# bharathikannann/Depth-Fusion-in-Transformer-Based-Video-Object-Detection

Hardware: AMD Instinct MI355X
Metric: frames/sec at 800x1333 RGB-D, TransVOD++ Late-Fusion (higher is better)
Workload: dtype f32; 1 GPU; TransVOD++ LateFusion, 32-frame 800x1333 RGB-D clip, all-current mode (R=31), L=1 DC5 (S=4200), 300 queries, 3 classes; frames_per_gpu=32, frames_per_gpu_per_clip=32, micro_batch=32, two_stream_overlap=False, clip_pipeline=True, pipeline_lanes=2, hip_hw_queues=4, hip_graphs=False

## Files before the change

### depth-fusion-in-transformer-based-video-object-detection_amd/csrc/conv_tile.hip

```cpp
#include "dfx_common.h"
#include "dfx_conv.h"
#include <type_traits>

namespace {

using f32x16 = __attribute__((ext_vector_type(16))) float;
using f32x4 = __attribute__((ext_vector_type(4))) float;
using i32x4 = __attribute__((ext_vector_type(4))) int;

constexpr int kTH = 8, kTW = 32, kThreads = 512, kMaxStage = 9;

struct TileArgs {
    const float *X, *Wp, *bias;
    float *Y;
    int Ci, H, W, Co, Ho, Wo, Kpad, K, KH, KW, stride, pad, act;
    long strideX, strideY;
    int TX, TY;
    long tiles;
    int IH, IW, PW;
    int nstage;
    unsigned xbytes;
};

__device__ __forceinline__ float activate(float v, int act)
// ... 13 lines not shown
    int *const koff = reinterpret_cast<int *>(smem + 32 * MT * LDA);
    float *const img = smem + 32 * MT * LDA + g.Kpad;
    float *const bl = img + 2 * IMG;

    const int tid = threadIdx.x, lane = tid & 63, wave = tid >> 6;
    const int half = lane >> 5, c = lane & 31;
    const int s = g.stride, PW = g.PW, PWH = PW >> 1;
    const int HW = g.H * g.W;

    for (int f = tid; f < 32 * MT * (g.Kpad / 4); f += kThreads) {
        const int row = f / (g.Kpad / 4), kq = f - row * (g.Kpad / 4);
        f32x4 v = {0.f, 0.f, 0.f, 0.f};
        if (row < g.Co) v = *reinterpret_cast<const f32x4 *>(g.Wp + (long)row * g.Kpad + kq * 4);
        *reinterpret_cast<f32x4 *>(As + row * LDA + kq * 4) = v;
    }
    for (int i = tid; i < 32 * MT; i += kThreads) bl[i] = (g.bias && i < g.Co) ? g.bias[i] : 0.f;
    for (int k = tid; k < g.Kpad; k += kThreads) {
        int o = 0;
        if (k < g.K) {
            const int tap = k / g.Ci, ci = k - tap * g.Ci, ky = tap / g.KW, kx = tap - ky * g.KW;
            o = ci * g.IH * PW + ky * PW + (s == 2 ? (kx & 1) * PWH + (kx >> 1) : kx);
        }
        koff[k] = o;
    }
    const int py = wave, px = c;
    const int pixbase = py * s * PW + px;

    int s_lds[NS], s_rx[NS];
    const int nel = g.Ci * g.IH * g.IW;
#pragma unroll
    for (int u = 0; u < NS; ++u) {
        const int e = tid + u * kThreads;
        const int ci = e / (g.IH * g.IW), rem = e - ci * (g.IH * g.IW), r = rem / g.IW, x = rem - r * g.IW;
        s_lds[u] = e < nel ? ci * g.IH * PW + r * PW + (s == 2 ? (x & 1) * PWH + (x >> 1) : x) : -1;
        s_rx[u] = (ci << 16) | (r << 8) | x;
    }
    const __amdgpu_buffer_rsrc_t rsX = __builtin_amdgcn_make_buffer_rsrc(const_cast<float *>(g.X), 0, (int)g.xbytes, 0x00020000);
    constexpr unsigned kOut = 0xFFFFFFFCu;
    float st[NS];
    const int G = (int)gridDim.x;
    const int d_n = G / (g.TY * g.TX), d_ty = (G - d_n * (g.TY * g.TX)) / g.TX, d_tx = G - d_n * (g.TY * g.TX) - d_ty * g.TX;
    struct Pos { int n, ty, tx; };
    auto advance = [&](Pos p) {
        p.tx += d_tx;
        if (p.tx >= g.TX) { p.tx -= g.TX; p.ty += 1; }
        p.ty += d_ty;
        if (p.ty >= g.TY) { p.ty -= g.TY; p.n += 1; }
        p.n += d_n;
        return p;
    };
    auto stage_load = [&](const Pos &p) {
        const int iy0 = p.ty * kTH * s - g.pad, ix0 = p.tx * kTW * s - g.pad;
        const int base = (int)((long)p.n * g.strideX) + iy0 * g.W + ix0;
        const bool inside = iy0 >= 0 && ix0 >= 0 && iy0 + g.IH <= g.H && ix0 + g.IW <= g.W;
        auto loads = [&](auto checked_tag) {
            constexpr bool CHECKED = decltype(checked_tag)::value;
#pragma unroll
            for (int u = 0; u < NS; ++u) {
                int pk = s_rx[u];
                asm volatile("" : "+v"(pk));
                const int x = pk & 255, r = (pk >> 8) & 255, ci = pk >> 16;
                unsigned off = (unsigned)(base + (ci * HW + r * g.W + x)) * 4u;
                bool bad = s_lds[u] < 0;
                if (CHECKED) bad = bad | ((unsigned)(ix0 + x) >= (unsigned)g.W) | ((unsigned)(iy0 + r) >= (unsigned)g.H);
                off = bad ? kOut : off;
                st[u] = __builtin_bit_cast(float, __builtin_amdgcn_raw_buffer_load_b32(rsX, off, 0, 0));
            }
        };
        if (inside) loads(std::false_type{}); else loads(std::true_type{});
    };
    auto stage_store = [&](int buf) {
        float *dst = img + buf * IMG;
#pragma unroll
        for (int u = 0; u < NS; ++u)
            if (s_lds[u] >= 0) dst[s_lds[u]] = st[u];
    };

    Pos cur;
    {
        const int t0 = (int)blockIdx.x, per = g.TY * g.TX;
        cur.n = t0 / per;
        cur.ty = (t0 - cur.n * per) / g.TX;
        cur.tx = t0 - cur.n * per - cur.ty * g.TX;
    }
    long t = blockIdx.x;
    if (t < g.tiles) {
        stage_load(cur);
        stage_store(0);
    }
    __syncthreads();
    const int nsteps = g.Kpad / 16;
    const unsigned P4 = (unsigned)(g.Ho * g.Wo) * 4u;
    int buf = 0;
    for (; t < g.tiles; t += G) {
        const bool more = t + G < g.tiles;
        const Pos nxt = advance(cur);
        if (more) stage_load(nxt);
        f32x16 acc[MT];
#pragma unroll
        for (int i = 0; i < MT; ++i)
#pragma unroll
            for (int r = 0; r < 16; ++r) acc[i][r] = bl[i * 32 + (r & 3) + 8 * (r >> 2) + 4 * half];
        const float *im = img + buf * IMG + pixbase;
#pragma unroll 1
        for (int ks = 0; ks < nsteps; ++ks) {
            const i32x4 o0 = *reinterpret_cast<const i32x4 *>(koff + ks * 16 + half * 4);
            const i32x4 o1 = *reinterpret_cast<const i32x4 *>(koff + ks * 16 + 8 + half * 4);
            f32x4 af[2][MT];
#pragma unroll
            for (int j = 0; j < 2; ++j)
#pragma unroll
                for (int i = 0; i < MT; ++i)
                    af[j][i] = *reinterpret_cast<const f32x4 *>(As + (i * 32 + c) * LDA + ks * 16 + j * 8 + half * 4);
            float bv[8];
#pragma unroll
            for (int q = 0; q < 4; ++q) {
                bv[q] = im[o0[q]];
                bv[4 + q] = im[o1[q]];
            }
#pragma unroll
            for (int q = 0; q < 8; ++q)
#pragma unroll
                for (int i = 0; i < MT; ++i)
                    acc[i] = __builtin_amdgcn_mfma_f32_32x32x2f32(af[q >> 2][i][q & 3], bv[q], acc[i], 0, 0, 0);
        }
        {
            const int oy = cur.ty * kTH + py, ox = cur.tx * kTW + px;
            const __amdgpu_buffer_rsrc_t rsY = __builtin_amdgcn_make_buffer_rsrc(g.Y + (long)cur.n * g.strideY, 0, (int)((unsigned)g.Co * P4), 0x00020000);
            const unsigned pix = (oy < g.Ho && ox < g.Wo) ? (unsigned)(oy * g.Wo + ox) * 4u + (unsigned)(4 * half) * P4 : 0x80000000u;
            auto write = [&](auto act_tag) {
                constexpr int ACT = decltype(act_tag)::value;
#pragma unroll
                for (int i = 0; i < MT; ++i)
#pragma unroll
                    for (int r = 0; r < 16; ++r) {
                        const int cr = i * 32 + (r & 3) + 8 * (r >> 2);
                        float v = acc[i][r];
                        if (ACT == DFX_ACT_RELU) asm("v_max_f32 %0, 0, %1" : "=v"(v) : "v"(v));
                        if (ACT == DFX_ACT_GELU) v = activate(v, DFX_ACT_GELU);
                        __builtin_amdgcn_raw_buffer_store_b32(__builtin_bit_cast(unsigned, v), rsY, pix, (unsigned)cr * P4, 0);
                    }
            };
            if (g.act == DFX_ACT_RELU) write(std::integral_constant<int, DFX_ACT_RELU>{});
            else if (g.act == DFX_ACT_GELU) write(std::integral_constant<int, DFX_ACT_GELU>{});
            else write(std::integral_constant<int, DFX_ACT_NONE>{});
        }
        if (more) stage_store(buf ^ 1);
        __syncthreads();
        buf ^= 1;
        cur = nxt;
    }
}

}

extern "C" int dfx_conv2d_tile_fits(int Ci, int Co, int KH, int KW, int stride, int dilation)
{
    if (Ci <= 0 || Co <= 0 || KH <= 0 || KW <= 0) return 0;
    const int K = Ci * KH * KW, Kpad = (K + 15) / 16 * 16;
    const int IH = (kTH - 1) * stride + KH, IW = (kTW - 1) * stride + KW;
    return (stride == 1 || stride == 2) && dilation == 1 && Co <= 64 && Kpad <= 160 && IH <= 255 && IW <= 255 &&
           (Ci * IH * IW + kThreads - 1) / kThreads <= kMaxStage;
}

extern "C" int dfx_conv2d_tile_f32(const float *x, const float *wp, const float *bias, float *y, int N, int Ci, int H, int W,
                                   int Co, int Ho, int Wo, int Kpad, int KH, int KW, int stride, int pad, int act,
                                   long x_image_stride, void *stream)
{
    if (N < 0 || Ci <= 0 || H <= 0 || W <= 0 || Co <= 0 || Ho < 0 || Wo < 0 || Kpad <= 0 || stride <= 0 || pad < 0 || KH <= 0 ||
        KW <= 0)
        return dfx::fail(DFX_EINVAL, "conv2d_tile: bad dimension");
    if ((long)N * Ho * Wo == 0) return DFX_OK;
    if (!x || !wp || !y) return dfx::fail(DFX_EINVAL, "conv2d_tile: null pointer");
    if (act < 0 || act > 2) return dfx::fail(DFX_EINVAL, "conv2d_tile: unknown activation");
    const int K = Ci * KH * KW;
    if (!dfx_conv2d_tile_fits(Ci, Co, KH, KW, stride, 1) || Kpad != (K + 15) / 16 * 16 || !dfx::aligned16(wp))
        return dfx::fail(DFX_EINVAL, "conv2d_tile: covers stride 1 / 2, Co <= 64, Ci * KH * KW <= 160 (padded to 16), wp 16-byte aligned");
    if ((Ho - 1) * stride - pad + KH > H + pad || (Wo - 1) * stride - pad + KW > W + pad)
        return dfx::fail(DFX_EINVAL, "conv2d_tile: output size does not match the input geometry");
    TileArgs g{};
    g.X = x; g.Wp = wp; g.bias = bias; g.Y = y;
    g.Ci = Ci; g.H = H; g.W = W; g.Co = Co; g.Ho = Ho; g.Wo = Wo; g.Kpad = Kpad; g.K = K; g.KH = KH; g.KW = KW;
    g.stride = stride; g.pad = pad; g.act = act;
    g.strideX = x_image_stride > 0 ? x_image_stride : (long)Ci * H * W;
    g.strideY = (long)Co * Ho * Wo;
    const long xel = (long)(N - 1) * g.strideX + (long)Ci * H * W;
    if (xel * 4 >= (1L << 32) - 8 || (long)Co * Ho * Wo * 4 >= (1L << 32))
        return dfx::fail(DFX_ERANGE, "conv2d_tile: the input batch or one output image exceeds 4 GiB (split the batch)");
    g.xbytes = (unsigned)(xel * 4);
    g.TY = (Ho + kTH - 1) / kTH;
    g.TX = (Wo + kTW - 1) / kTW;
    g.tiles = (long)N * g.TY * g.TX;
    g.IH = (kTH - 1) * stride + KH;
    g.IW = (kTW - 1) * stride + KW;
    g.PW = stride == 2 ? 2 * ((g.IW + 1) / 2) : g.IW;
    g.nstage = (Ci * g.IH * g.IW + kThreads - 1) / kThreads;
    const int MT = Co <= 32 ? 1 : 2;
    const size_t lds = (size_t)(32 * MT * (Kpad + 4) + Kpad + 2 * Ci * g.IH * g.PW + 32 * MT) * 4;
    if (lds > 160 * 1024) return dfx::fail(DFX_EINVAL, "conv2d_tile: the staged tile does not fit the LDS");
    hipStream_t st = static_cast<hipStream_t>(stream);
    static std::mutex mu;
    static bool raised_on[64] = {false};
    int dev = 0;
    (void)hipGetDevice(&dev);
    {
        std::lock_guard<std::mutex> lock(mu);
        if (!raised_on[dev & 63]) {
            if (hipFuncSetAttribute(reinterpret_cast<const void *>(&conv_tile_kernel<1, 3>), hipFuncAttributeMaxDynamicSharedMemorySize, 160 * 1024) != hipSuccess ||
                hipFuncSetAttribute(reinterpret_cast<const void *>(&conv_tile_kernel<1, kMaxStage>), hipFuncAttributeMaxDynamicSharedMemorySize, 160 * 1024) != hipSuccess ||
                hipFuncSetAttribute(reinterpret_cast<const void *>(&conv_tile_kernel<2, kMaxStage>), hipFuncAttributeMaxDynamicSharedMemorySize, 160 * 1024) != hipSuccess)
                return dfx::fail(DFX_ELAUNCH, "conv2d_tile: cannot raise the dynamic LDS limit");
            raised_on[dev & 63] = true;
        }
    }
    static int ncu = 0;
    if (ncu == 0) {
        int n = 0;
        if (hipDeviceGetAttribute(&n, hipDeviceAttributeMultiprocessorCount, dev) != hipSuccess || n < 8) n = 256;
        ncu = n;
    }
    const long per_cu = lds * 4 <= 160 * 1024 ? 4 : lds * 2 <= 160 * 1024 ? 2 : 1;
    const long grid = g.tiles < ncu * per_cu ? g.tiles : ncu * per_cu;
    const long flops = 2L * Co * Kpad * Ho * Wo * N;
    if (MT == 1 && g.nstage <= 3) dfx::launch_timed(flops, -4, 16, conv_tile_kernel<1, 3>, dim3((unsigned)grid), dim3(kThreads), lds, st, g);
    else if (MT == 1) dfx::launch_timed(flops, -4, 16, conv_tile_kernel<1, kMaxStage>, dim3((unsigned)grid), dim3(kThreads), lds, st, g);
    else dfx::launch_timed(flops, -4, 16, conv_tile_kernel<2, kMaxStage>, dim3((unsigned)grid), dim3(kThreads), lds, st, g);
    return dfx::check_launch("conv_tile_kernel");
}
```

### depth-fusion-in-transformer-based-video-object-detection_amd/dfx/_lib.py

```python
import ctypes
import os

_HERE = os.path.dirname(os.path.abspath(__file__))
_SO = os.environ.get("DFX_LIBRARY") or os.path.join(_HERE, "libdfx.so")
_lib = None

_i, _l, _p = ctypes.c_int, ctypes.c_long, ctypes.c_void_p
_DIMS = [_i] * 7

SIGNATURES = {
    "dfx_msda_forward_f32": [_p] * 5 + _DIMS + [_p, _p],
    "dfx_msda_forward_f64": [_p] * 5 + _DIMS + [_p, _p],
    "dfx_msda_backward_f32": [_p] * 6 + _DIMS + [_p, _p, _p, _p],
    "dfx_msda_backward_f64": [_p] * 6 + _DIMS + [_p, _p, _p, _p],
    "dfx_msda_forward_bf16": [_p] * 5 + _DIMS + [_p, _p],
    "dfx_msda_forward_f16": [_p] * 5 + _DIMS + [_p, _p],
    "dfx_msda_backward_bf16": [_p] * 6 + _DIMS + [_p, _p, _p, _p],
    "dfx_msda_backward_f16": [_p] * 6 + _DIMS + [_p, _p, _p, _p],
    "dfx_msda_fused_forward_f32": [_p, _p, _p, _p, _i, _i, _p, _l, _p, _l] + _DIMS + [_p, _p],
    "dfx_msda_fused_backward_f32": [_p, _p, _p, _p, _i, _p, _l, _p, _l, _p] + _DIMS + [_p, _p, _l, _p, _l, _p, _p],
    "dfx_msda_level_grad_value_f32": [_p, _i, _p, _l, _p, _l, _p, _i, _i, _i, _i, _p, _p],
    "dfx_profile_enable": [_i],
    "dfx_tuning_reload": [],
    "dfx_profile_drain": [_p, _p, _p, _p, _i],
    "dfx_msda_fused_level_fits": [_i, _i],
    "dfx_msda_fused_level_forward_f32": [_p, _p, _i, _p, _p, _p, _i, _i, _i, _i, _p, _p],
    "dfx_mha_f32": [_p, _l, _l, _p, _l, _l, _p, _l, _l, _p, _l, _l, _i, _i, _i, _i, ctypes.c_float, _p],
    "dfx_mha_train_forward_f32": [_p, _l, _l] * 4 + [_p, _p, _i, _i, _i, _i, ctypes.c_float, _p],
    "dfx_mha_backward_f32": [_p, _l, _l] * 5 + [_p, _p] + [_p, _l, _l] * 3 + [_i, _i, _i, _i, ctypes.c_float, _p],
    "dfx_roi_align_nchw_f32": [_p, _p] + [_i] * 7 + [ctypes.c_float, _i, _i, _p, _p],
    "dfx_roi_align_nhwc_f32": [_p, _p] + [_i] * 7 + [ctypes.c_float, _i, _i, _p, _p],
    "dfx_roi_align_backward_nchw_f32": [_p, _p] + [_i] * 7 + [ctypes.c_float, _i, _i, _p, _p],
    "dfx_roi_align_backward_nhwc_f32": [_p, _p] + [_i] * 7 + [ctypes.c_float, _i, _i, _p, _p],
    "dfx_dynamic_conv_f32": [_p, _p, _l, _p, _p, _p, _p, _p, _i, _i, _i, _i, ctypes.c_float, _p],
    "dfx_dynamic_conv_backward_f32": [_p, _p, _p, _l, _p, _p, _p, _p, _p, _p, _l, _p, _p, _i, _i, _i, _i, ctypes.c_float, _p],
    "dfx_preprocess_u8_f32": [_p, _i, _i, _i, _p, _p, _i, _p, _p, _i, _i, _i, _p, _p, _p, _l, _i, _i, _p, _p],
    "dfx_gemm_f32": [_p, _p, _l, _l, _p, _l, _l, _i, _p, _i, _p, _l, _l, _p, _l, _p, _l, _l, _i, _i, _i, _i, _i, _i, _l, _l, _p],
    "dfx_gemm_splitk_f32": [_p, _l, _p, _l, _i, _p, _i, _p, _l, _p, _l, _i, _i, _i, _i, _i, _p, _p],
    "dfx_conv1x1_pair_f32": [_p, _p, _l, _i, _p, _l, _i, _p, _p, _l, _i, _i, _i, _i, _p],
    "dfx_conv1x1_chain_f32": [_p, _p, _l, _i, _p, _l, _i, _p, _p, _l, _p, _l, _p, _p, _p, _l, _i, _i, _i, _i, _i, _p],
    "dfx_bias_act_nchw_f32": [_p, _p, _p, _p, _i, _i, _l, _i, _p],
    "dfx_bias_relu_maxpool_f32": [_p, _p, _p, _i, _i, _i, _i, _p],
    "dfx_add_layernorm_f32": [_p, _p, _p, _p, _p, _l, _i, ctypes.c_float, _p],
    "dfx_box_refine_f32": [_p, _p, _i, _p, _l, ctypes.c_float, _p],
    "dfx_group_norm_f32": [_p, _p, _p, _p, _p, _i, _i, _l, _i, ctypes.c_float, _i, _p],
    "dfx_conv2d_igemm_f32": [_p, _p, _p, _p, _p] + [_i] * 14 + [_l, _p],
    "dfx_conv2d_tile_fits": [_i] * 6,
    "dfx_conv2d_tile_f32": [_p, _p, _p, _p] + [_i] * 13 + [_l, _p],
    "dfx_conv3x3_wino_f32": [_p, _p, _p, _p] + [_i] * 7 + [_p],
    "dfx_wino_weights_f32": [_p, _p, _p, _i, _i, _p],
}


class LevelLayout(ctypes.Structure):
    _fields_ = [(n, ctypes.c_long) for n in (
        "value_frame", "value_token", "value_head", "value_oct", "value_chunk",
        "off_row", "off_head", "logit_row", "logit_head",
        "out_row", "out_head", "out_oct", "out_chunk")]


def library_path():
    return _SO


def load():
    global _lib
    if _lib is None:
        if not os.path.exists(_SO):
            raise RuntimeError(
                f"{_SO} is missing: the HIP extension has not been built "
                "(run `python __graft_entry__.py build` or `make -C <pkg>/csrc`). "
                "There is no CPU or PyTorch fallback for this operator.")
        lib = ctypes.CDLL(_SO)
        for name, argtypes in SIGNATURES.items():
            fn = getattr(lib, name)
            fn.argtypes = argtypes
            fn.restype = ctypes.c_int
        lib.dfx_abi_version.restype = ctypes.c_int
        lib.dfx_last_error.restype = ctypes.c_char_p
        _lib = lib
    return _lib


def abi_version():
    return load().dfx_abi_version()


def check(rc, what):
    if rc != 0:
        msg = load().dfx_last_error().decode() or f"error code {rc}"
        raise RuntimeError(f"{what}: {msg}")
```

### depth-fusion-in-transformer-based-video-object-detection_amd/dfx/ops.py

```python
import ctypes
import os

import torch

from . import _lib

_SUFFIX = {torch.float32: "f32", torch.float64: "f64"}
_HALF_SUFFIX = {torch.bfloat16: "bf16", torch.float16: "f16"}
ACT = {None: 0, "none": 0, "relu": 1, "gelu": 2}

USE_LEVEL_KERNEL = os.environ.get("DFX_MSDA_LEVEL", "1") == "1"
LEVEL_MIN_QUERIES = 1024
USE_LEVEL_BWD = os.environ.get("DFX_MSDA_LEVEL_BWD", "1") != "0"
LEVEL_BWD_MIN_QUERIES = 9600
USE_TILE_CONV = os.environ.get("DFX_TILE_CONV", "1") == "1"

def profile_start():
    _lib.load().dfx_profile_enable(1)


def reload_tuning():
    _lib.load().dfx_tuning_reload()


# ... 713 lines not shown
    @staticmethod
    def forward(ctx, q, k, v, drop, heads, scale):
        out, lse = mha_train_forward(q, k, v, heads, scale, drop)
        ctx.heads, ctx.scale = heads, scale
        ctx.save_for_backward(q, k, v, out, lse, drop)
        return out

    @staticmethod
    @torch.autograd.function.once_differentiable
    def backward(ctx, grad_output):
        q, k, v, out, lse, drop = ctx.saved_tensors
        need = ctx.needs_input_grad
        gq, gk, gv = mha_backward(grad_output.contiguous(), q, k, v, out, lse, ctx.heads, ctx.scale, drop, need_q=need[0],
                                  need_kv=need[1] or need[2])
        return gq, gk if need[1] else None, gv if need[2] else None, None, None, None


def mha(q, k, v, heads, scale, drop=None):
    if torch.is_grad_enabled() and (q.requires_grad or k.requires_grad or v.requires_grad):
        _mha_checks(q, k, v, heads)
        return _MhaFunction.apply(q, k, v, drop, heads, float(scale))
    if drop is not None:
        return mha_train_forward(q, k, v, heads, scale, drop)[0]
    B, Lq, Lk, E = _mha_checks(q, k, v, heads)
    out = torch.empty((B, Lq, E), dtype=torch.float32, device=q.device)
    _call("mha", "dfx_mha_f32", q.device, q.data_ptr(), q.stride(0), q.stride(1), k.data_ptr(), k.stride(0), k.stride(1),
          v.data_ptr(), v.stride(0), v.stride(1), out.data_ptr(), Lq * E, E, B, heads, Lq, Lk, float(scale))
    return out


def box_refine(delta, reference, eps=1e-5):
    delta, reference = delta.contiguous(), reference.contiguous()
    _check_inputs([("delta", delta), ("reference", reference)])
    rd = reference.shape[-1]
    _require(delta.shape[-1] == 4 and rd in (2, 4) and delta.shape[:-1] == reference.shape[:-1]
             and delta.dtype == torch.float32 and reference.dtype == torch.float32,
             "box_refine: delta [...,4], reference [...,2|4], fp32")
    out = torch.empty_like(delta)
    _call("box_refine", "dfx_box_refine_f32", delta.device, delta.data_ptr(), reference.data_ptr(), rd, out.data_ptr(),
          delta.numel() // 4, float(eps))
    return out


def add_layernorm(x, residual, norm):
    C = x.shape[-1]
    x2 = x.contiguous()
    named = [("x", x2), ("weight", norm.weight), ("bias", norm.bias)]
    if residual is not None:
        residual = residual.contiguous()
        named.append(("residual", residual))
        _require(residual.shape == x2.shape, "residual must match x")
    _check_inputs(named)
    _require(x2.dtype == torch.float32 and norm.weight.numel() == C, "add_layernorm: fp32, LayerNorm over the last dim")
    out = torch.empty_like(x2)
    _call("add_layernorm", "dfx_add_layernorm_f32", x2.device, x2.data_ptr(), _ptr(residual), norm.weight.data_ptr(),
          norm.bias.data_ptr(), out.data_ptr(), x2.numel() // C, C, float(norm.eps))
    return out


def bias_relu_maxpool(x, bias):
    _check_inputs([("x", x), ("bias", bias)])
    _require(x.dtype == torch.float32 and x.dim() == 4 and bias.numel() == x.shape[1], "bias_relu_maxpool: fp32 NCHW")
    N, C, H, W = x.shape
    out = torch.empty((N, C, (H + 1) // 2, (W + 1) // 2), dtype=x.dtype, device=x.device)
    _call("bias_relu_maxpool", "dfx_bias_relu_maxpool_f32", x.device, x.data_ptr(), bias.data_ptr(), out.data_ptr(), N, C, H, W)
    return out


class ConvPlan:
    WINO_MAX_ELEMENTS = 1 << 30

    def __init__(self, weight, bias=None, stride=1, padding=0, dilation=1, act=None, scale=None, algo=None, groups=1,
                 padding_mode="zeros"):
        _require(weight.is_cuda and weight.dtype == torch.float32 and weight.dim() == 4, "ConvPlan: fp32 CUDA weight [Co,Ci,kh,kw]")
        for nm, v in (("stride", stride), ("padding", padding), ("dilation", dilation)):
            _require(not isinstance(v, (tuple, list)) or len(set(int(e) for e in v)) == 1,
                     f"ConvPlan: {nm} must be the same along both axes (got {tuple(v) if isinstance(v, (tuple, list)) else v})")
        stride, padding, dilation = (v[0] if isinstance(v, (tuple, list)) else v for v in (stride, padding, dilation))
        Co, Ci, kh, kw = weight.shape
        _require(groups == 1 and padding_mode == "zeros", "ConvPlan: grouped convolutions / non-zero padding modes are not covered")
        _require(kh <= 32 and kw <= 32, "ConvPlan: kernel sides up to 32")
        self.Co, self.Ci, self.kh, self.kw = Co, Ci, kh, kw
        self.stride, self.padding, self.dilation, self.act = int(stride), int(padding), int(dilation), ACT[act]
        self.bias = None if bias is None else bias.detach().float().contiguous()
        wino_ok = kh == 3 and kw == 3 and stride == 1 and padding == dilation and Ci % 8 == 0 and Co % 64 == 0
        tile_ok = bool(_lib.load().dfx_conv2d_tile_fits(Ci, Co, kh, kw, int(stride), int(dilation)))
        self.algo = algo or ("wino" if wino_ok else "tile" if (tile_ok and Ci <= 4 and USE_TILE_CONV) else "igemm")
        _require(self.algo != "wino" or wino_ok, "ConvPlan: geometry not covered by the Winograd kernel")
        _require(self.algo != "tile" or tile_ok, "ConvPlan: geometry not covered by the tile kernel")
        w = weight.detach().contiguous()
        if self.algo == "wino":
            self.u = torch.empty(16 * Co * Ci, dtype=torch.float32, device=w.device)
            sc = None if scale is None else scale.detach().float().contiguous()
            _call("wino_weights", "dfx_wino_weights_f32", w.device, w.data_ptr(), _ptr(sc), self.u.data_ptr(), Co, Ci)
        else:
            if scale is not None:
                w = w * scale.detach().reshape(-1, 1, 1, 1)
            K = kh * kw * Ci
            Kpad = (K + 15) // 16 * 16
            _require(kh * kw <= 64, "ConvPlan: at most 64 taps")
            wp = torch.zeros(Co, Kpad, dtype=torch.float32, device=w.device)
            wp[:, :K] = w.permute(0, 2, 3, 1).reshape(Co, K)
            self.wp, self.Kpad, self.K, self._tabs = wp, Kpad, K, {}

    def _ktab(self, H, W, device):
        key = (H, W, str(device))
        if key not in self._tabs:
            ky, kx, ci = torch.meshgrid(torch.arange(self.kh), torch.arange(self.kw), torch.arange(self.Ci), indexing="ij")
            tab = torch.zeros((self.Kpad, 2), dtype=torch.int32)
            tab[:, 0] = -1
            tab[:self.K, 0] = (ky * self.kw + kx).reshape(-1).to(torch.int32)
            tab[:self.K, 1] = ((ci * (H * W) + ky * self.dilation * W + kx * self.dilation) * 4).reshape(-1).to(torch.int32)
            self._tabs[key] = tab.to(device)
        return self._tabs[key]

    def out_size(self, H, W):
        eff_h, eff_w = (self.kh - 1) * self.dilation + 1, (self.kw - 1) * self.dilation + 1
        return (H + 2 * self.padding - eff_h) // self.stride + 1, (W + 2 * self.padding - eff_w) // self.stride + 1

    def __call__(self, x):
        _require(x.is_cuda and x.dtype == torch.float32 and x.dim() == 4 and x.shape[1] == self.Ci,
                 "conv: x must be a CUDA fp32 tensor [N,Ci,H,W] (no CPU path)")
        N, _, H, W = x.shape
        sliced = (self.algo in ("igemm", "tile") and not x.is_contiguous() and x.stride(3) == 1 and x.stride(2) == W
                  and x.stride(1) == H * W and x.stride(0) >= self.Ci * H * W)
        image_stride = x.stride(0) if sliced else 0
        if not sliced:
            x = x.contiguous()
        Ho, Wo = self.out_size(H, W)
        y = torch.empty((N, self.Co, Ho, Wo), dtype=torch.float32, device=x.device)
        step = N
        if self.algo == "wino" and N * self.Ci * H * W >= self.WINO_MAX_ELEMENTS:
            step = max(1, (self.WINO_MAX_ELEMENTS - 1) // (self.Ci * H * W))
        if self.algo == "tile":
            step = max(1, min(N, ((1 << 30) - 4) // max(image_stride, self.Ci * H * W)))
        with _on(x.device):
            for n0 in range(0, N, step):
                n1 = min(N, n0 + step)
                xs, ys = x[n0:n1], y[n0:n1]
                if self.algo == "wino":
                    _call("conv wino", "dfx_conv3x3_wino_f32", x.device, xs.data_ptr(), self.u.data_ptr(), _ptr(self.bias),
                          ys.data_ptr(), n1 - n0, self.Ci, H, W, self.Co, self.dilation, self.act)
                elif self.algo == "tile":
                    _call("conv tile", "dfx_conv2d_tile_f32", x.device, xs.data_ptr(), self.wp.data_ptr(), _ptr(self.bias),
                          ys.data_ptr(), n1 - n0, self.Ci, H, W, self.Co, Ho, Wo, self.Kpad, self.kh, self.kw, self.stride,
                          self.padding, self.act, image_stride)
                else:
                    _call("conv igemm", "dfx_conv2d_igemm_f32", x.device, xs.data_ptr(), self.wp.data_ptr(),
                          self._ktab(H, W, x.device).data_ptr(), _ptr(self.bias), ys.data_ptr(), n1 - n0, self.Ci, H, W, self.Co,
                          Ho, Wo, self.Kpad, self.kh, self.kw, self.stride, self.padding, self.dilation, self.act, image_stride)
        return y


def group_norm(x, norm, tokens_out=False):
    _check_inputs([("x", x), ("weight", norm.weight), ("bias", norm.bias)])
    _require(x.dtype == torch.float32 and x.dim() == 4 and x.shape[1] == norm.num_channels, "group_norm: fp32 NCHW")
    N, C, H, W = x.shape
    stats = torch.empty(N * norm.num_groups * 2, dtype=torch.float32, device=x.device)
    y = torch.empty((N, H * W, C) if tokens_out else (N, C, H, W), dtype=torch.float32, device=x.device)
    _call("group_norm", "dfx_group_norm_f32", x.device, x.data_ptr(), norm.weight.data_ptr(), norm.bias.data_ptr(),
          stats.data_ptr(), y.data_ptr(), N, C, H * W, norm.num_groups, float(norm.eps), int(bool(tokens_out)))
    return y.transpose(1, 2).unflatten(2, (H, W)) if tokens_out else y
```

### depth-fusion-in-transformer-based-video-object-detection_amd/models/resnet.py

```python
import torch
from torch import nn

import os

from dfx import ops as _ops

_PAIR_SHORTCUT = os.environ.get("DFX_PAIR_SHORTCUT", "1") == "1"
_CONV_CHAIN = os.environ.get("DFX_CONV_CHAIN", "1") == "1"
_CONV_CHAIN_MAX_C1 = int(os.environ.get("DFX_CONV_CHAIN_MAX_C1", "128"))


def _fold(conv, bn):
    scale, shift = bn.scale_shift()
    return (conv.weight.detach() * scale.reshape(-1, 1, 1, 1)).contiguous(), shift.detach().contiguous()


def _versions(*mods):
    out = []
    for m in mods:
        for t in list(m.parameters(recurse=False)) + list(m.buffers(recurse=False)):
            out.append((t.data_ptr(), t._version))
    return tuple(out)


class Bottleneck(nn.Module):
    expansion = 4

    def __init__(self, inplanes, planes, stride, dilation, downsample, norm_layer):
        super().__init__()
        self.conv1 = nn.Conv2d(inplanes, planes, 1, bias=False)
        self.bn1 = norm_layer(planes)
        self.conv2 = nn.Conv2d(planes, planes, 3, stride=stride, padding=dilation, dilation=dilation, bias=False)
        self.bn2 = norm_layer(planes)
        self.conv3 = nn.Conv2d(planes, planes * 4, 1, bias=False)
        self.bn3 = norm_layer(planes * 4)
        self.relu = nn.ReLU(inplace=True)
        self.downsample = downsample
        self._folded = None

    def _folded_params(self):
        mods = [self.conv1, self.bn1, self.conv2, self.bn2, self.conv3, self.bn3]
        if self.downsample is not None:
            mods += [self.downsample[0], self.downsample[1]]
        key = _versions(*mods)
        if self._folded is None or self._folded[0] != key:
            c2 = self.conv2
            scale2, shift2 = self.bn2.scale_shift()
            plan2 = _ops.ConvPlan(c2.weight, shift2.detach(), c2.stride, c2.padding, c2.dilation, "relu",
                                  scale=scale2.detach(), groups=c2.groups, padding_mode=c2.padding_mode)
            f = [_fold(self.conv1, self.bn1), plan2, _fold(self.conv3, self.bn3)]
            f.append(_fold(self.downsample[0], self.downsample[1]) if self.downsample is not None else None)
            pair = None
            if self.downsample is not None and self.downsample[0].stride[0] == 1 and _PAIR_SHORTCUT:
                (w3, b3), (wd, bd) = f[2], f[3]
                if w3.shape[1] % 16 == 0 and wd.shape[1] % 16 == 0:
                    pair = (torch.cat([w3.flatten(1), wd.flatten(1)], 1).contiguous(), (b3 + bd).contiguous())
            f.append(pair)
            self._folded = (key, f)
        return self._folded[1]

    def chain_conv1(self):
        c = self.conv1
        if c.kernel_size != (1, 1) or c.stride != (1, 1) or c.padding != (0, 0) or c.groups != 1:
            return None
        return self._folded_params()[0]

    def forward_fused(self, x, z=None, nxt=None):
        (w1, b1), plan2, (w3, b3), down, pair = self._folded_params()
        out = z if z is not None else self._conv1x1(0, x, w1, b1, relu=True)
        out = plan2(out)
        hw = out.shape[2] * out.shape[3]
        chain = nxt is not None and hw % 4 == 0 and nxt[0].shape[0] <= _CONV_CHAIN_MAX_C1
        if pair is not None and hw % 4 == 0 and out.shape[2:] == x.shape[2:]:
            if chain and _ops.conv1x1_chain_supported(pair[0].shape[0], out.shape[1], x.shape[1], nxt[0].shape[0], hw):
                return _ops.conv1x1_chain(out, pair[0], pair[1], nxt[0], nxt[1], x2=x.contiguous())
            y = _ops.conv1x1_pair(out, x.contiguous(), pair[0], pair[1], relu=True)
            return y if nxt is None else (y, None)
        if down is not None:
            x = self._conv1x1(1, x, down[0], down[1], relu=False, stride=self.downsample[0].stride[0])
        if chain and _ops.conv1x1_chain_supported(w3.shape[0], out.shape[1], 0, nxt[0].shape[0], hw):
            return _ops.conv1x1_chain(out, w3, b3, nxt[0], nxt[1], residual=x)
        y = self._conv1x1(2, out, w3, b3, relu=True, residual=x)
        return y if nxt is None else (y, None)

    def _conv1x1(self, slot, x, w, b, relu, residual=None, stride=1):
        ho, wo = (x.shape[2] + stride - 1) // stride, (x.shape[3] + stride - 1) // stride
        if (ho * wo) % 4 == 0 and stride == 1:
            return _ops.conv1x1(x, w, b, residual=residual, relu=relu, stride=stride)
        key = self._folded[0]
        plans = self.__dict__.setdefault("_plans1x1", {})
        fused = residual is None
        if slot not in plans or plans[slot][0] != key:
            plans[slot] = (key, _ops.ConvPlan(w.reshape(w.shape[0], -1, 1, 1), b if fused else None, stride, 0, 1,
                                              "relu" if (fused and relu) else None))
        y = plans[slot][1](x)
        return y if fused else _ops.bias_act_(y, b, residual=residual, relu=relu)

    def forward(self, x):
        out = self.relu(self.bn1(self.conv1(x)))
        out = self.relu(self.bn2(self.conv2(out)))
        out = self.bn3(self.conv3(out))
        skip = x if self.downsample is None else self.downsample(x)
        return self.relu(out + skip)


class ResNet50(nn.Module):
    def __init__(self, norm_layer, replace_stride_with_dilation=(False, False, False)):
        super().__init__()
        self.inplanes, self.dilation = 64, 1
        self.conv1 = nn.Conv2d(3, 64, 7, stride=2, padding=3, bias=False)
        self.bn1 = norm_layer(64)
        self.relu = nn.ReLU(inplace=True)
        self.maxpool = nn.MaxPool2d(3, stride=2, padding=1)
        self.layer1 = self._stage(64, 3, 1, False, norm_layer)
        self.layer2 = self._stage(128, 4, 2, replace_stride_with_dilation[0], norm_layer)
        self.layer3 = self._stage(256, 6, 2, replace_stride_with_dilation[1], norm_layer)
        self.layer4 = self._stage(512, 3, 2, replace_stride_with_dilation[2], norm_layer)
        self.avgpool = nn.AdaptiveAvgPool2d((1, 1))
        self.fc = nn.Linear(2048, 1000)
        for m in self.modules():
            if isinstance(m, nn.Conv2d):
                nn.init.kaiming_normal_(m.weight, mode="fan_out", nonlinearity="relu")

    def _stage(self, planes, blocks, stride, dilate, norm_layer):
        first_dilation = self.dilation
        if dilate:
            self.dilation *= stride
            stride = 1
        downsample = None
        if stride != 1 or self.inplanes != planes * 4:
            downsample = nn.Sequential(nn.Conv2d(self.inplanes, planes * 4, 1, stride=stride, bias=False),
                                       norm_layer(planes * 4))
        layers = [Bottleneck(self.inplanes, planes, stride, first_dilation, downsample, norm_layer)]
        self.inplanes = planes * 4
        for _ in range(1, blocks):
            layers.append(Bottleneck(self.inplanes, planes, 1, self.dilation, None, norm_layer))
        return nn.Sequential(*layers)

    def stem(self, x, fused=False):
        if not fused:
            return self.maxpool(self.relu(self.bn1(self.conv1(x))))
        key = _versions(self.conv1, self.bn1)
        if getattr(self, "_stem_folded", None) is None or self._stem_folded[0] != key:
            scale, shift = self.bn1.scale_shift()
            self._stem_folded = (key, (_ops.ConvPlan(self.conv1.weight, None, 2, 3, 1, None, scale=scale.detach()),
                                       shift.detach().contiguous()))
        plan, b = self._stem_folded[1]
        return _ops.bias_relu_maxpool(plan(x), b)

    def run_stage(self, stage, x, fused=False):
        if not fused:
            return stage(x)
        carry, self._chain_carry = self.__dict__.get("_chain_carry"), None
        z = carry[1] if carry is not None and carry[0] is x else None
        follower = {id(self.layer1): self.layer2, id(self.layer2): self.layer3}.get(id(stage)) if _CONV_CHAIN else None
        blocks = list(stage)
        for i, block in enumerate(blocks):
            succ = None
            if follower is not None:
                succ = blocks[i + 1] if i + 1 < len(blocks) else follower[0]
            nxt = succ.chain_conv1() if succ is not None else None
            if nxt is None:
                x, z = block.forward_fused(x, z), None
            else:
                x, z = block.forward_fused(x, z, nxt)
        if z is not None:
            self._chain_carry = (x, z)
        return x

    def forward(self, x):
        x = self.stem(x)
        return self.layer4(self.layer3(self.layer2(self.layer1(x))))
```

### include/dfx_conv.h

```cpp
#ifndef DFX_CONV_H
#define DFX_CONV_H

#ifdef __cplusplus
extern "C" {
#endif

#define DFX_ACT_NONE 0
#define DFX_ACT_RELU 1
#define DFX_ACT_GELU 2

int dfx_conv2d_igemm_f32(const float *x, const float *wp, const int *ktab, const float *bias, float *y,
                         int N, int Ci, int H, int W, int Co, int Ho, int Wo, int Kpad, int KH, int KW,
                         int stride, int pad, int dilation, int act, long x_image_stride, void *stream);

int dfx_conv2d_tile_fits(int Ci, int Co, int KH, int KW, int stride, int dilation);
int dfx_conv2d_tile_f32(const float *x, const float *wp, const float *bias, float *y,
                        int N, int Ci, int H, int W, int Co, int Ho, int Wo, int Kpad, int KH, int KW,
                        int stride, int pad, int act, long x_image_stride, void *stream);

int dfx_conv3x3_wino_f32(const float *x, const float *u, const float *bias, float *y,
                         int N, int Ci, int H, int W, int Co, int dilation, int act, void *stream);

int dfx_wino_weights_f32(const float *w, const float *scale, float *u, int Co, int Ci, void *stream);

#ifdef __cplusplus
}
#endif
#endif
```

Baseline: 399.0 frames/s.

## Fuse stem conv, BN shift, ReLU and 3x3 maxpool into one tiled kernel

Result: no change. 401.4 frames/s, median of 6 (+0.6%).

```diff
diff --git a/depth-fusion-in-transformer-based-video-object-detection_amd/csrc/conv_tile.hip b/depth-fusion-in-transformer-based-video-object-detection_amd/csrc/conv_tile.hip
--- a/depth-fusion-in-transformer-based-video-object-detection_amd/csrc/conv_tile.hip
+++ b/depth-fusion-in-transformer-based-video-object-detection_amd/csrc/conv_tile.hip
@@ -189,6 +189,212 @@
     }
 }
 
+constexpr int kPoolCols = 15, kPoolSlots = 2 * kPoolCols;
+
+struct PoolArgs {
+    const float *X, *Wp, *shift;
+    float *Y;
+    int Ci, H, W, Co, Ho, Wo, Kpad, K, KH, KW, stride, pad;
+    int PHo, PWo;
+    long strideX, strideY;
+    int S, TY;
+    long tiles, per;
+    int IH, IW, PW;
+    unsigned xbytes;
+};
+
+__device__ __forceinline__ float lane_up(float v)
+{
+    return __builtin_bit_cast(float, __builtin_amdgcn_update_dpp(__builtin_bit_cast(int, v), __builtin_bit_cast(int, v), 0x130, 0xf, 0xf, false));
+}
+
+template <int NS>
+__global__ __launch_bounds__(kThreads, 4) void conv_tile_pool_kernel(const PoolArgs g)
+{
+    constexpr int MT = 2;
+    extern __shared__ __attribute__((aligned(16))) float smem[];
+    const long first = (long)blockIdx.x * g.per, last = first + g.per < g.tiles ? first + g.per : g.tiles;
+    if (first >= last) return;
+    const int LDA = g.Kpad + 4;
+    const int IMG = g.Ci * g.IH * g.PW;
+    float *const As = smem;
+    int *const koff = reinterpret_cast<int *>(smem + 32 * MT * LDA);
+    float *const img = smem + 32 * MT * LDA + g.Kpad;
+    float *const carry = img + 2 * IMG;
+
+    const int tid = threadIdx.x, lane = tid & 63, wave = tid >> 6;
+    const int half = lane >> 5, c = lane & 31;
+    const int s = g.stride, PW = g.PW, PWH = PW >> 1;
+    const int HW = g.H * g.W;
+
+    for (int f = tid; f < 32 * MT * (g.Kpad / 4); f += kThreads) {
+        const int row = f / (g.Kpad / 4), kq = f - row * (g.Kpad / 4);
+        f32x4 v = {0.f, 0.f, 0.f, 0.f};
+        if (row < g.Co) v = *reinterpret_cast<const f32x4 *>(g.Wp + (long)row * g.Kpad + kq * 4);
+        *reinterpret_cast<f32x4 *>(As + row * LDA + kq * 4) = v;
+    }
+    for (int i = tid; i < 32 * MT; i += kThreads) As[i * LDA + g.Kpad] = i < g.Co ? g.shift[i] : 0.f;
+    for (int k = tid; k < g.Kpad; k += kThreads) {
+        int o = 0;
+        if (k < g.K) {
+            const int tap = k / g.Ci, ci = k - tap * g.Ci, ky = tap / g.KW, kx = tap - ky * g.KW;
+            o = ci * g.IH * PW + ky * PW + (s == 2 ? (kx & 1) * PWH + (kx >> 1) : kx);
+        }
+        koff[k] = o;
+    }
+    const int pixbase = wave * s * PW + c;
+
+    int s_lds[NS], s_rx[NS];
+    const int nel = g.Ci * g.IH * g.IW;
+#pragma unroll
+    for (int u = 0; u < NS; ++u) {
+        const int e = tid + u * kThreads;
+        const int ci = e / (g.IH * g.IW), rem = e - ci * (g.IH * g.IW), r = rem / g.IW, x = rem - r * g.IW;
+        s_lds[u] = e < nel ? ci * g.IH * PW + r * PW + (s == 2 ? (x & 1) * PWH + (x >> 1) : x) : -1;
+        s_rx[u] = (ci << 16) | (r << 8) | x;
+    }
+    const __amdgpu_buffer_rsrc_t rsX = __builtin_amdgcn_make_buffer_rsrc(const_cast<float *>(g.X), 0, (int)g.xbytes, 0x00020000);
+    constexpr unsigned kOut = 0xFFFFFFFCu;
+    float st[NS];
+    struct Pos { int n, sj, t; };
+    auto advance = [&](Pos p) {
+        p.t += 1;
+        if (p.t >= g.TY) { p.t = 0; p.sj += 1; }
+        if (p.sj >= g.S) { p.sj = 0; p.n += 1; }
+        return p;
+    };
+    auto stage_load = [&](const Pos &p) {
+        const int iy0 = p.t * kTH * s - g.pad, ix0 = (p.sj * 2 * kPoolCols - 1) * s - g.pad;
+        const int base = (int)((long)p.n * g.strideX) + iy0 * g.W + ix0;
+        const bool inside = iy0 >= 0 && ix0 >= 0 && iy0 + g.IH <= g.H && ix0 + g.IW <= g.W;
+        auto loads = [&](auto checked_tag) {
+            constexpr bool CHECKED = decltype(checked_tag)::value;
+#pragma unroll
+            for (int u = 0; u < NS; ++u) {
+                int pk = s_rx[u];
+                asm volatile("" : "+v"(pk));
+                const int x = pk & 255, r = (pk >> 8) & 255, ci = pk >> 16;
+                unsigned off = (unsigned)(base + (ci * HW + r * g.W + x)) * 4u;
+                bool bad = s_lds[u] < 0;
+                if (CHECKED) bad = bad | ((unsigned)(ix0 + x) >= (unsigned)g.W) | ((unsigned)(iy0 + r) >= (unsigned)g.H);
+                off = bad ? kOut : off;
+                st[u] = __builtin_bit_cast(float, __builtin_amdgcn_raw_buffer_load_b32(rsX, off, 0, 0));
+            }
+        };
+        if (inside) loads(std::false_type{}); else loads(std::true_type{});
+    };
+    auto stage_store = [&](int buf) {
+        float *dst = img + buf * IMG;
+#pragma unroll
+        for (int u = 0; u < NS; ++u)
+            if (s_lds[u] >= 0) dst[s_lds[u]] = st[u];
+    };
+
+    Pos cur;
+    {
+        const long per_img = (long)g.S * g.TY;
+        cur.n = (int)(first / per_img);
+        const int rem = (int)(first - cur.n * per_img);
+        cur.sj = rem / g.TY;
+        cur.t = rem - cur.sj * g.TY;
+    }
+    long idx = first;
+    if (cur.t > 0) { cur.t -= 1; idx -= 1; }
+    stage_load(cur);
+    stage_store(0);
+    __syncthreads();
+    const int nsteps = g.Kpad / 16;
+    const unsigned PP4 = (unsigned)(g.PHo * g.PWo) * 4u;
+    const bool keeper = !(c & 1) && c < 2 * kPoolCols;
+    const int slot = half * kPoolCols + (c >> 1);
+    int buf = 0;
+    for (; idx < last; ++idx) {
+        const bool more = idx + 1 < last;
+        const Pos nxt = advance(cur);
+        if (more) stage_load(nxt);
+        f32x16 acc[MT];
+#pragma unroll
+        for (int i = 0; i < MT; ++i)
+#pragma unroll
+            for (int r = 0; r < 16; ++r) acc[i][r] = 0.f;
+        const float *im = img + buf * IMG + pixbase;
+#pragma unroll 1
+        for (int ks = 0; ks < nsteps; ++ks) {
+            const i32x4 o0 = *reinterpret_cast<const i32x4 *>(koff + ks * 16 + half * 4);
+            const i32x4 o1 = *reinterpret_cast<const i32x4 *>(koff + ks * 16 + 8 + half * 4);
+            f32x4 af[2][MT];
+#pragma unroll
+            for (int j = 0; j < 2; ++j)
+#pragma unroll
+                for (int i = 0; i < MT; ++i)
+                    af[j][i] = *reinterpret_cast<const f32x4 *>(As + (i * 32 + c) * LDA + ks * 16 + j * 8 + half * 4);
+            float bv[8];
+#pragma unroll
+            for (int q = 0; q < 4; ++q) {
+                bv[q] = im[o0[q]];
+                bv[4 + q] = im[o1[q]];
+            }
+#pragma unroll
+            for (int q = 0; q < 8; ++q)
+#pragma unroll
+                for (int i = 0; i < MT; ++i)
+                    acc[i] = __builtin_amdgcn_mfma_f32_32x32x2f32(af[q >> 2][i][q & 3], bv[q], acc[i], 0, 0, 0);
+        }
+        const int oy = cur.t * kTH + wave, ox0 = cur.sj * 2 * kPoolCols - 1;
+        if (ox0 < 0 || ox0 + kTW > g.Wo || cur.t * kTH + kTH > g.Ho) {
+            const bool in_map = oy < g.Ho && (unsigned)(ox0 + c) < (unsigned)g.Wo;
+#pragma unroll
+            for (int i = 0; i < MT; ++i)
+#pragma unroll
+                for (int r = 0; r < 16; ++r) acc[i][r] = in_map ? acc[i][r] : -INFINITY;
+        }
+#pragma unroll
+        for (int i = 0; i < MT; ++i)
+#pragma unroll
+            for (int r = 0; r < 16; ++r) {
+                const float v1 = lane_up(acc[i][r]), v2 = lane_up(v1);
+                acc[i][r] = fmaxf(fmaxf(acc[i][r], v1), v2);
+            }
+        if (wave == 0 && cur.t > 0 && keeper) {
+#pragma unroll
+            for (int q = 0; q < 16 * MT; ++q) acc[q >> 4][q & 15] = fmaxf(acc[q >> 4][q & 15], carry[q * kPoolSlots + slot]);
+        }
+        __syncthreads();
+        float *const xch = img + buf * IMG;
+        if ((wave & 1) && keeper) {
+#pragma unroll
+            for (int q = 0; q < 16 * MT; ++q) xch[((wave >> 1) * 16 * MT + q) * kPoolSlots + slot] = acc[q >> 4][q & 15];
+            if (wave == kTH - 1) {
+#pragma unroll
+                for (int q = 0; q < 16 * MT; ++q) carry[q * kPoolSlots + slot] = acc[q >> 4][q & 15];
+            }
+        }
+        if (more) stage_store(buf ^ 1);
+        __syncthreads();
+        if (!(wave & 1) && idx >= first) {
+            const int p = wave >> 1, prow = cur.t * (kTH / 2) + p, pcol = cur.sj * kPoolCols + (c >> 1);
+            const __amdgpu_buffer_rsrc_t rsY = __builtin_amdgcn_make_buffer_rsrc(g.Y + (long)cur.n * g.strideY, 0, (int)((unsigned)g.Co * PP4), 0x00020000);
+            const unsigned pix = (keeper && prow < g.PHo && pcol < g.PWo) ? (unsigned)(prow * g.PWo + pcol) * 4u + (unsigned)(4 * half) * PP4 : 0x80000000u;
+            const float *const xhi = xch + p * 16 * MT * kPoolSlots + (keeper ? slot : 0);
+            const float *const xlo = p > 0 ? xhi - 16 * MT * kPoolSlots : xhi;
+            const float *const sh = As + 4 * half * LDA + g.Kpad;
+#pragma unroll
+            for (int q0 = 0; q0 < 16 * MT; q0 += 8) {
+#pragma unroll
+                for (int q = q0; q < q0 + 8; ++q) {
+                    const int cr = (q >> 4) * 32 + (q & 3) + 8 * ((q & 15) >> 2);
+                    float v = fmaxf(fmaxf(acc[q >> 4][q & 15], xhi[q * kPoolSlots]), xlo[q * kPoolSlots]) + sh[cr * LDA];
+                    asm("v_max_f32 %0, 0, %1" : "=v"(v) : "v"(v));
+                    __builtin_amdgcn_raw_buffer_store_b32(__builtin_bit_cast(unsigned, v), rsY, pix, (unsigned)cr * PP4, 0);
+                }
+                __builtin_amdgcn_sched_barrier(0);
+            }
+        }
+        buf ^= 1;
+        cur = nxt;
+    }
+}
+
 }
 
 extern "C" int dfx_conv2d_tile_fits(int Ci, int Co, int KH, int KW, int stride, int dilation)
@@ -198,6 +404,74 @@
     const int IH = (kTH - 1) * stride + KH, IW = (kTW - 1) * stride + KW;
     return (stride == 1 || stride == 2) && dilation == 1 && Co <= 64 && Kpad <= 160 && IH <= 255 && IW <= 255 &&
            (Ci * IH * IW + kThreads - 1) / kThreads <= kMaxStage;
+}
+
+extern "C" int dfx_conv2d_tile_pool_fits(int Ci, int Co, int KH, int KW, int stride, int dilation)
+{
+    if (!dfx_conv2d_tile_fits(Ci, Co, KH, KW, stride, dilation) || Co <= 32) return 0;
+    const int IH = (kTH - 1) * stride + KH, IW = (kTW - 1) * stride + KW, PW = stride == 2 ? 2 * ((IW + 1) / 2) : IW;
+    const int K = Ci * KH * KW, Kpad = (K + 15) / 16 * 16, img = Ci * IH * PW;
+    return img >= (kTH / 2) * 32 * kPoolSlots && (64 * (Kpad + 4) + Kpad + 2 * img + 32 * kPoolSlots) * 4 <= 80 * 1024;
+}
+
+extern "C" int dfx_conv2d_tile_pool_f32(const float *x, const float *wp, const float *shift, float *y, int N, int Ci, int H,
+                                        int W, int Co, int Ho, int Wo, int Kpad, int KH, int KW, int stride, int pad,
+                                        long x_image_stride, int max_workgroups, void *stream)
+{
+    if (N < 0 || Ci <= 0 || H <= 0 || W <= 0 || Co <= 0 || Ho < 0 || Wo < 0 || Kpad <= 0 || stride <= 0 || pad < 0 || KH <= 0 ||
+        KW <= 0 || max_workgroups < 0)
+        return dfx::fail(DFX_EINVAL, "conv2d_tile_pool: bad dimension");
+    if ((long)N * Ho * Wo == 0) return DFX_OK;
+    if (!x || !wp || !shift || !y) return dfx::fail(DFX_EINVAL, "conv2d_tile_pool: null pointer");
+    const int K = Ci * KH * KW;
+    if (!dfx_conv2d_tile_pool_fits(Ci, Co, KH, KW, stride, 1) || Kpad != (K + 15) / 16 * 16 || !dfx::aligned16(wp))
+        return dfx::fail(DFX_EINVAL, "conv2d_tile_pool: covers the tile kernel's geometries with 32 < Co <= 64 whose staged tile holds the pooling exchange, wp 16-byte aligned");
+    if ((Ho - 1) * stride - pad + KH > H + pad || (Wo - 1) * stride - pad + KW > W + pad)
+        return dfx::fail(DFX_EINVAL, "conv2d_tile_pool: output size does not match the input geometry");
+    PoolArgs g{};
+    g.X = x; g.Wp = wp; g.shift = shift; g.Y = y;
+    g.Ci = Ci; g.H = H; g.W = W; g.Co = Co; g.Ho = Ho; g.Wo = Wo; g.Kpad = Kpad; g.K = K; g.KH = KH; g.KW = KW;
+    g.stride = stride; g.pad = pad;
+    g.PHo = (Ho + 1) / 2; g.PWo = (Wo + 1) / 2;
+    g.strideX = x_image_stride > 0 ? x_image_stride : (long)Ci * H * W;
+    g.strideY = (long)Co * g.PHo * g.PWo;
+    const long xel = (long)(N - 1) * g.strideX + (long)Ci * H * W;
+    if (xel * 4 >= (1L << 32) - 8 || (long)Co * Ho * Wo * 4 >= (1L << 31))
+        return dfx::fail(DFX_ERANGE, "conv2d_tile_pool: the input batch exceeds 4 GiB or one output image 2 GiB (split the batch)");
+    g.xbytes = (unsigned)(xel * 4);
+    g.TY = (Ho + kTH - 1) / kTH;
+    g.S = (g.PWo + kPoolCols - 1) / kPoolCols;
+    g.tiles = (long)N * g.S * g.TY;
+    g.IH = (kTH - 1) * stride + KH;
+    g.IW = (kTW - 1) * stride + KW;
+    g.PW = stride == 2 ? 2 * ((g.IW + 1) / 2) : g.IW;
+    const size_t lds = (size_t)(64 * (Kpad + 4) + Kpad + 2 * Ci * g.IH * g.PW + 32 * kPoolSlots) * 4;
+    hipStream_t st = static_cast<hipStream_t>(stream);
+    static std::mutex mu;
+    static bool raised_on[64] = {false};
+    static int ncu = 0;
+    int dev = 0;
+    (void)hipGetDevice(&dev);
+    {
+        std::lock_guard<std::mutex> lock(mu);
+        if (!raised_on[dev & 63]) {
+            if (hipFuncSetAttribute(reinterpret_cast<const void *>(&conv_tile_pool_kernel<kMaxStage>), hipFuncAttributeMaxDynamicSharedMemorySize, 80 * 1024) != hipSuccess)
+                return dfx::fail(DFX_ELAUNCH, "conv2d_tile_pool: cannot raise the dynamic LDS limit");
+            raised_on[dev & 63] = true;
+        }
+        if (ncu == 0) {
+            int n = 0;
+            if (hipDeviceGetAttribute(&n, hipDeviceAttributeMultiprocessorCount, dev) != hipSuccess || n < 8) n = 256;
+            ncu = n;
+        }
+    }
+    long grid = g.tiles < 2L * ncu ? g.tiles : 2L * ncu;
+    if (max_workgroups > 0 && grid > max_workgroups) grid = max_workgroups;
+    g.per = (g.tiles + grid - 1) / grid;
+    grid = (g.tiles + g.per - 1) / g.per;
+    const long flops = 2L * Co * Kpad * Ho * Wo * N;
+    dfx::launch_timed(flops, -4, 17, conv_tile_pool_kernel<kMaxStage>, dim3((unsigned)grid), dim3(kThreads), lds, st, g);
+    return dfx::check_launch("conv_tile_pool_kernel");
 }
 
 extern "C" int dfx_conv2d_tile_f32(const float *x, const float *wp, const float *bias, float *y, int N, int Ci, int H, int W,
diff --git a/depth-fusion-in-transformer-based-video-object-detection_amd/dfx/_lib.py b/depth-fusion-in-transformer-based-video-object-detection_amd/dfx/_lib.py
--- a/depth-fusion-in-transformer-based-video-object-detection_amd/dfx/_lib.py
+++ b/depth-fusion-in-transformer-based-video-object-detection_amd/dfx/_lib.py
@@ -47,6 +47,8 @@
     "dfx_conv2d_igemm_f32": [_p, _p, _p, _p, _p] + [_i] * 14 + [_l, _p],
     "dfx_conv2d_tile_fits": [_i] * 6,
     "dfx_conv2d_tile_f32": [_p, _p, _p, _p] + [_i] * 13 + [_l, _p],
+    "dfx_conv2d_tile_pool_fits": [_i] * 6,
+    "dfx_conv2d_tile_pool_f32": [_p, _p, _p, _p] + [_i] * 12 + [_l, _i, _p],
     "dfx_conv3x3_wino_f32": [_p, _p, _p, _p] + [_i] * 7 + [_p],
     "dfx_wino_weights_f32": [_p, _p, _p, _i, _i, _p],
 }
diff --git a/depth-fusion-in-transformer-based-video-object-detection_amd/dfx/ops.py b/depth-fusion-in-transformer-based-video-object-detection_amd/dfx/ops.py
--- a/depth-fusion-in-transformer-based-video-object-detection_amd/dfx/ops.py
+++ b/depth-fusion-in-transformer-based-video-object-detection_amd/dfx/ops.py
@@ -889,6 +889,37 @@
         return y
 
 
+def conv_relu_maxpool_supported(plan, x):
+    if plan.algo != "tile" or plan.bias is not None or plan.act != ACT[None] or x.dim() != 4:
+        return False
+    if not _lib.load().dfx_conv2d_tile_pool_fits(plan.Ci, plan.Co, plan.kh, plan.kw, plan.stride, plan.dilation):
+        return False
+    N, _, H, W = x.shape
+    Ho, Wo = plan.out_size(H, W)
+    return Ho > 0 and Wo > 0 and N * max(x.stride(0), plan.Ci * H * W) < (1 << 30) - 4 and plan.Co * Ho * Wo * 4 < (1 << 31)
+
+
+def conv_relu_maxpool(plan, x, shift, max_workgroups=0):
+    _require(x.is_cuda and x.dtype == torch.float32 and x.dim() == 4 and x.shape[1] == plan.Ci and shift.dtype == torch.float32
+             and shift.numel() == plan.Co, "conv_relu_maxpool: CUDA fp32 x [N,Ci,H,W], shift [Co] (no CPU path)")
+    N, _, H, W = x.shape
+    sliced = (not x.is_contiguous() and x.stride(3) == 1 and x.stride(2) == W and x.stride(1) == H * W
+              and x.stride(0) >= plan.Ci * H * W)
+    image_stride = x.stride(0) if sliced else 0
+    if not sliced:
+        x = x.contiguous()
+    _check_inputs([("shift", shift), ("weights", plan.wp)] + ([] if sliced else [("x", x)]))
+    _require(x.device == shift.device, "conv_relu_maxpool: x and shift on different devices")
+    _require(conv_relu_maxpool_supported(plan, x), "conv_relu_maxpool: plan / map not covered by the fused kernel")
+    Ho, Wo = plan.out_size(H, W)
+    y = torch.empty((N, plan.Co, (Ho + 1) // 2, (Wo + 1) // 2), dtype=torch.float32, device=x.device)
+    with _on(x.device):
+        _call("conv tile pool", "dfx_conv2d_tile_pool_f32", x.device, x.data_ptr(), plan.wp.data_ptr(), shift.data_ptr(),
+              y.data_ptr(), N, plan.Ci, H, W, plan.Co, Ho, Wo, plan.Kpad, plan.kh, plan.kw, plan.stride, plan.padding,
+              image_stride, int(max_workgroups))
+    return y
+
+
 def group_norm(x, norm, tokens_out=False):
     _check_inputs([("x", x), ("weight", norm.weight), ("bias", norm.bias)])
     _require(x.dtype == torch.float32 and x.dim() == 4 and x.shape[1] == norm.num_channels, "group_norm: fp32 NCHW")
diff --git a/depth-fusion-in-transformer-based-video-object-detection_amd/models/resnet.py b/depth-fusion-in-transformer-based-video-object-detection_amd/models/resnet.py
--- a/depth-fusion-in-transformer-based-video-object-detection_amd/models/resnet.py
+++ b/depth-fusion-in-transformer-based-video-object-detection_amd/models/resnet.py
@@ -8,6 +8,7 @@
 _PAIR_SHORTCUT = os.environ.get("DFX_PAIR_SHORTCUT", "1") == "1"
 _CONV_CHAIN = os.environ.get("DFX_CONV_CHAIN", "1") == "1"
 _CONV_CHAIN_MAX_C1 = int(os.environ.get("DFX_CONV_CHAIN_MAX_C1", "128"))
+_STEM_POOL = os.environ.get("DFX_STEM_POOL", "1") == "1"
 
 
 def _fold(conv, bn):
@@ -146,6 +147,8 @@
             self._stem_folded = (key, (_ops.ConvPlan(self.conv1.weight, None, 2, 3, 1, None, scale=scale.detach()),
                                        shift.detach().contiguous()))
         plan, b = self._stem_folded[1]
+        if _STEM_POOL and _ops.conv_relu_maxpool_supported(plan, x):
+            return _ops.conv_relu_maxpool(plan, x, b)
         return _ops.bias_relu_maxpool(plan(x), b)
 
     def run_stage(self, stage, x, fused=False):
diff --git a/include/dfx_conv.h b/include/dfx_conv.h
--- a/include/dfx_conv.h
+++ b/include/dfx_conv.h
@@ -18,6 +18,11 @@
                         int N, int Ci, int H, int W, int Co, int Ho, int Wo, int Kpad, int KH, int KW,
                         int stride, int pad, int act, long x_image_stride, void *stream);
 
+int dfx_conv2d_tile_pool_fits(int Ci, int Co, int KH, int KW, int stride, int dilation);
+int dfx_conv2d_tile_pool_f32(const float *x, const float *wp, const float *shift, float *y,
+                             int N, int Ci, int H, int W, int Co, int Ho, int Wo, int Kpad, int KH, int KW,
+                             int stride, int pad, long x_image_stride, int max_workgroups, void *stream);
+
 int dfx_conv3x3_wino_f32(const float *x, const float *u, const float *bias, float *y,
                          int N, int Ci, int H, int W, int Co, int dilation, int act, void *stream);
 
```
